# excamera/alfalfa

Hardware: NVIDIA H100
Metric: decode_throughput (higher is better)
Workload: dtype u8

## Files before the change

### alfalfa_b200/csrc/tokens.cu

```cuda
#include <cuda_runtime.h>
#include <stdint.h>
#include <stdlib.h>

#include "engine.h"
#include "tokens_core.cuh"

namespace vp8 {
namespace {

constexpr int kMaxCols = 1024;
template <int kTokWarps>
__global__ void __launch_bounds__(32 * kTokWarps) k_tokens(const uint8_t* ring, size_t stride, int first, int count,
                                                          int nslots, Geom g) {
  __shared__ __align__(16) uint8_t probs_all[kTokWarps][tok::kProbBytes];
  __shared__ uint16_t above_all[kTokWarps][kMaxCols];
  const int warp = threadIdx.x >> 5, lane = threadIdx.x & 31;
  const int job = blockIdx.x * kTokWarps + warp;
  if (job >= count) return;
  uint8_t* probs = probs_all[warp];
  uint16_t* above_nz = above_all[warp];
  const TokJob& J = *reinterpret_cast<const TokJob*>(ring + static_cast<size_t>((first + job) % nslots) * stride);
  for (int e = lane; e < tok::kProbEntries; e += 32) tok::expand_prob_entry(J.coef_probs, probs, e);
  for (int i = lane; i < g.mb_cols; i += 32) above_nz[i] = 0;
  __syncwarp();
  if (lane != 0) return;
  tok::decode_frame_tokens(J, g, probs, above_nz);
}

__global__ void __launch_bounds__(32) k_tokens_lockstep(const uint8_t* ring, size_t stride, int first, int count,
                                                         int nslots, Geom g) {
#ifdef VP8GPU_SIMT_EMUL
  uint8_t* const dyn = simt::dyn_smem();
#else
  extern __shared__ __align__(16) uint8_t dyn[];
#endif
  __shared__ tok::LockstepTables T;
  uint8_t* const P = dyn;
  uint16_t* const above = reinterpret_cast<uint16_t*>(dyn + 1056 * 32);
  const int lane = threadIdx.x;
  tok::fill_lockstep_tables(T, lane, 32);
  const int job = blockIdx.x * 32 + lane;
  const TokJob* J = job < count ? reinterpret_cast<const TokJob*>(ring + static_cast<size_t>((first + job) % nslots) * stride) : nullptr;
  if (J) {
    const uint32_t* src = reinterpret_cast<const uint32_t*>(J->coef_probs);
    for (int w = 0; w < 264; w++) {
      const uint32_t v = __ldg(src + w);
      P[(4 * w + 0) * 32 + lane] = v & 0xFF;
      P[(4 * w + 1) * 32 + lane] = (v >> 8) & 0xFF;
      P[(4 * w + 2) * 32 + lane] = (v >> 16) & 0xFF;
      P[(4 * w + 3) * 32 + lane] = v >> 24;
    }
  }
  __syncwarp();
  if (!J) return;
  tok::decode_frame_tokens_lockstep<32>(*J, g, T, P + lane, above + lane);
}

}

int launch_tokens(const uint8_t* ring, size_t stride, int first, int count, int nslots, const Geom& g, void* stream) {
  if (g.mb_cols > kMaxCols) return (int)cudaErrorInvalidValue;
  static const int warps = [] {
    const char* v = getenv("VP8GPU_TOK_WARPS");
    return v && atoi(v) == 8 ? 8 : (v && atoi(v) == 32 ? 32 : 1);
  }();
  cudaStream_t s = static_cast<cudaStream_t>(stream);
  if (warps == 32) {
    const size_t smem = 1056 * 32 + (size_t)g.mb_cols * 32 * sizeof(uint16_t);
    static const cudaError_t attr = cudaFuncSetAttribute(k_tokens_lockstep, cudaFuncAttributeMaxDynamicSharedMemorySize, 1056 * 32 + kMaxCols * 64);
    if (attr != cudaSuccess) return (int)attr;
    VP8_LAUNCH(k_tokens_lockstep, (count + 31) / 32, 32, smem, s)(ring, stride, first, count, nslots, g);
  }
  else if (warps == 8) VP8_LAUNCH(k_tokens<8>, (count + 7) / 8, 256, 0, s)(ring, stride, first, count, nslots, g);
  else VP8_LAUNCH(k_tokens<1>, count, 32, 0, s)(ring, stride, first, count, nslots, g);
  return (int)cudaGetLastError();
}

}
```

### alfalfa_b200/csrc/tokens_core.cuh

```cuda
#pragma once
#include <stdint.h>

#include "engine.h"

#ifdef __CUDACC__
#define TK_DEV __device__ __forceinline__
#define TK_CONST __constant__
#define TK_LDG(p) __ldg(p)
#define TK_LDCG(p) __ldcg(p)
#define TK_CLZ(x) __clz(x)
#else
#define TK_DEV inline __attribute__((always_inline))
#define TK_CONST static const
#define TK_LDG(p) (*(p))
#define TK_LDCG(p) (*(p))
#define TK_CLZ(x) __builtin_clz(x)
#endif

namespace vp8 {
namespace tok {

TK_CONST uint8_t c_band[16] = {0, 1, 2, 3, 6, 4, 5, 6, 6, 6, 6, 6, 6, 6, 6, 7};
TK_CONST uint8_t c_zigzag[16] = {0, 1, 4, 8, 5, 2, 3, 6, 9, 12, 13, 10, 7, 11, 14, 15};
TK_CONST uint8_t c_cat[5][11] = {{165, 145},
                                 {173, 148, 140},
                                 {176, 155, 140, 135},
                                 {180, 157, 141, 134, 130},
                                 {254, 254, 243, 230, 196, 177, 153, 140, 133, 130, 129}};

constexpr int kProbEntries = 4 * 8 * 3;
constexpr int kProbBytes = kProbEntries * 16;
struct alignas(16) Probs16 {
  uint32_t w[4];
  TK_DEV uint32_t at(int k) const { return (w[k >> 2] >> ((k & 3) * 8)) & 0xFF; }
};
TK_DEV void expand_prob_entry(const uint8_t* src, uint8_t* dst, int e) {
  for (int k = 0; k < 11; k++) dst[e * 16 + k] = src[e * 11 + k];
  for (int k = 11; k < 16; k++) dst[e * 16 + k] = 0;
}

#ifdef __CUDACC__
#define TK_BSWAP(x) __byte_perm((x), 0, 0x0123)
#else
#define TK_BSWAP(x) __builtin_bswap32(x)
#endif
struct LaneReader {
  const uint8_t* p;
  const uint8_t* end;
  uint64_t value;
  int nbits;
  uint32_t nxt;
  uint32_t range;
};
TK_DEV uint32_t lr_fetch(LaneReader& b) {
  uint32_t w = 0;
  if (b.p + 4 <= b.end) {
    w = TK_BSWAP(TK_LDG(reinterpret_cast<const uint32_t*>(b.p)));
  } else {
    for (int k = 0; k < 4; k++)
      if (b.p + k < b.end) w |= static_cast<uint32_t>(TK_LDG(b.p + k)) << (24 - 8 * k);
  }
  b.p += 4;
  return w;
}
TK_DEV void lr_refill(LaneReader& b) {
  b.value |= static_cast<uint64_t>(b.nxt) << (32 - b.nbits);
  b.nbits += 32;
  b.nxt = lr_fetch(b);
}
TK_DEV void lr_init(LaneReader& b, const uint8_t* data, uint32_t n) {
  b.p = data;
  b.end = data + n;
  b.value = 0;
  b.nbits = 0;
  b.range = 255;
  while ((reinterpret_cast<uintptr_t>(b.p) & 3) && b.p < b.end) {
    b.value |= static_cast<uint64_t>(TK_LDG(b.p++)) << (56 - b.nbits);
    b.nbits += 8;
  }
  if (b.p >= b.end) b.p = reinterpret_cast<const uint8_t*>((reinterpret_cast<uintptr_t>(b.p) + 3) & ~static_cast<uintptr_t>(3));
  b.nxt = lr_fetch(b);
  lr_refill(b);
  if (b.nbits <= 32) lr_refill(b);
}
TK_DEV int lr_decide(LaneReader& b, uint32_t prob) {
  const uint32_t split = 1 + (((b.range - 1) * prob) >> 8);
  uint32_t hi = static_cast<uint32_t>(b.value >> 32);
  const uint32_t big = split << 24;
  const int bit = hi >= big;
  const uint32_t r = bit ? b.range - split : split;
  hi -= bit ? big : 0u;
  const int shift = TK_CLZ(r) - 24;
  b.range = r << shift;
  b.value = ((static_cast<uint64_t>(hi) << 32) | static_cast<uint32_t>(b.value)) << shift;
  b.nbits -= shift;
  return bit;
}
TK_DEV void lr_ensure(LaneReader& b) {
  if (b.nbits <= 32) lr_refill(b);
}
TK_DEV int lr_get(LaneReader& b, uint32_t prob) {
  const int bit = lr_decide(b, prob);
  lr_ensure(b);
  return bit;
}

constexpr uint64_t kBandNibbles = 0x7666666665463210ull;
TK_DEV uint32_t band_off(int i) {
  return static_cast<uint32_t>((kBandNibbles >> (4 * (i & 15))) & 15) * 48;
}
TK_DEV Probs16 ld_probs(const uint8_t* p) { return *reinterpret_cast<const Probs16*>(p); }

TK_DEV int parse_block(LaneReader& br, const uint8_t* tp, int ctx, int i, uint32_t tag, vp8gpu_token*& out) {
  lr_ensure(br);
  Probs16 P = ld_probs(tp + band_off(i) + ctx * 16);
  if (!lr_decide(br, P.at(0))) return 0;
  int nz = 0;
  for (;;) {
    lr_ensure(br);
    const uint32_t next = band_off(i + 1);
    const Probs16 Pz = ld_probs(tp + next);
    if (!lr_decide(br, P.at(1))) {
      if (++i == 16) return nz;
      P = Pz;
      continue;
    }
    int v;
    Probs16 Pn;
    if (!lr_decide(br, P.at(2))) {
      Pn = ld_probs(tp + next + 16);
      v = 1;
    } else {
      Pn = ld_probs(tp + next + 32);
      lr_ensure(br);
      if (!lr_decide(br, P.at(3))) {
        if (!lr_decide(br, P.at(4))) v = 2;
        else v = 3 + lr_decide(br, P.at(5));
      } else {
        int cat, n, base;
        if (!lr_decide(br, P.at(6))) {
          if (!lr_decide(br, P.at(7))) {
            cat = 0, n = 0, base = 5 + lr_decide(br, 159);
          } else {
            cat = 0, n = 2, base = 7;
          }
        } else if (!lr_decide(br, P.at(8))) {
          if (!lr_decide(br, P.at(9))) cat = 1, n = 3, base = 11;
          else cat = 2, n = 4, base = 19;
        } else {
          if (!lr_decide(br, P.at(10))) cat = 3, n = 5, base = 35;
          else cat = 4, n = 11, base = 67;
        }
        int inc = 0;
        for (int k = 0; k < n; k++) {
          lr_ensure(br);
          inc = (inc << 1) + lr_decide(br, c_cat[cat][k]);
        }
        v = base + inc;
      }
      lr_ensure(br);
    }
    if (lr_decide(br, 128)) v = -v;
    *out++ = tag | (static_cast<uint32_t>(c_zigzag[i]) << 16) | static_cast<uint16_t>(v);
    nz = 1;
    if (++i == 16) return 1;
    P = Pn;
    if (!lr_decide(br, P.at(0))) return 1;
  }
}

TK_DEV void decode_frame_tokens(const TokJob& J, const Geom& g, const uint8_t* probs, uint16_t* above_nz) {
  LaneReader parts[8];
  const int nparts = static_cast<int>(J.nparts);
  for (int i = 0; i < nparts; i++) lr_init(parts[i], J.bits + J.part_off[i], J.part_len[i]);

  vp8gpu_mb* const mbs = J.mbs;
  vp8gpu_token* const t_begin = J.tokens;
  vp8gpu_token* t = t_begin;
  const vp8gpu_token* const t_limit = t_begin + J.tok_cap;
  uint32_t overflow = 0;
  const uint8_t* const coef_y_after_y2 = probs + 0 * 384;
  const uint8_t* const coef_y2 = probs + 1 * 384;
  const uint8_t* const coef_uv = probs + 2 * 384;
  const uint8_t* const coef_y_full = probs + 3 * 384;

  const uint32_t* rec = reinterpret_cast<const uint32_t*>(mbs);
  uint32_t w1 = TK_LDCG(rec + 1), w2 = TK_LDCG(rec + 2);
  const int n_mbs = g.mb_cols * g.mb_rows;
  int idx = 0;
  for (int row = 0; row < g.mb_rows; row++) {
    unsigned left_nz = 0;
    LaneReader tr = parts[row & (nparts - 1)];
    for (int col = 0; col < g.mb_cols; col++, idx++) {
      const uint32_t cur1 = w1, cur2 = w2;
      if (idx + 1 < n_mbs) {
        w1 = TK_LDCG(rec + 8 * (idx + 1) + 1);
        w2 = TK_LDCG(rec + 8 * (idx + 1) + 2);
      }
      const int y_mode = (cur1 >> 16) & 0xFF;
      const bool skip = (cur2 >> 24) & VP8GPU_MB_SKIP;
      const bool has_y2 = y_mode != VP8GPU_B_PRED && y_mode != VP8GPU_SPLITMV;
      unsigned a_nz = above_nz[col];
      vp8gpu_token* const t0 = t;
      if (skip) {
        const unsigned keep = has_y2 ? 0u : 0x100u;
        a_nz &= keep;
        left_nz &= keep;
      } else if (t + 400 > t_limit) {
        overflow = 1;
        a_nz = 0;
        left_nz = 0;
      } else {
        const uint8_t* y_probs = coef_y_full;
        int first = 0;
        if (has_y2) {
          const int ctx = ((a_nz >> 8) & 1) + ((left_nz >> 8) & 1);
          const unsigned nz = parse_block(tr, coef_y2, ctx, 0, VP8GPU_BLK_Y2 << 20, t);
          a_nz = (a_nz & ~0x100u) | (nz << 8);
          left_nz = (left_nz & ~0x100u) | (nz << 8);
          y_probs = coef_y_after_y2;
          first = 1;
        }
#pragma unroll 1
        for (int b = 0; b < 24; b++) {
          int bx, by;
          const uint8_t* tp;
          int f;
          if (b < 16) {
            bx = b & 3, by = b >> 2, tp = y_probs, f = first;
          } else {
            const int sh = 4 + 2 * ((b - 16) >> 2);
            bx = sh + (b & 1), by = sh + ((b >> 1) & 1), tp = coef_uv, f = 0;
          }
          const int ctx = ((a_nz >> bx) & 1) + ((left_nz >> by) & 1);
          const unsigned nz = parse_block(tr, tp, ctx, f, static_cast<uint32_t>(b) << 20, t);
          a_nz = (a_nz & ~(1u << bx)) | (nz << bx);
          left_nz = (left_nz & ~(1u << by)) | (nz << by);
        }
      }
      above_nz[col] = static_cast<uint16_t>(a_nz);
      uint32_t* wr = reinterpret_cast<uint32_t*>(mbs) + 8 * idx;
      wr[0] = static_cast<uint32_t>(t0 - t_begin);
      wr[1] = (cur1 & 0xFFFF0000u) | static_cast<uint32_t>(t - t0);
      wr[2] = cur2 & ~(static_cast<uint32_t>(VP8GPU_MB_SKIP) << 24);
    }
    parts[row & (nparts - 1)] = tr;
  }
  J.result[0] = static_cast<uint32_t>(t - t_begin);
  if (overflow) J.result[1] = 1;
}


constexpr int kNodeExtra = 11, kNodeSign = 12, kNodeEnd = 13;
#define TK_T(next, setv, zero, cat) static_cast<uint16_t>((next) | ((setv) << 4) | ((zero) << 8) | ((cat) << 9))
TK_CONST uint16_t c_trans[22] = {
    TK_T(kNodeEnd, 0, 0, 0),  TK_T(1, 0, 0, 0),
    TK_T(1, 0, 1, 0),         TK_T(2, 0, 0, 0),
    TK_T(kNodeSign, 1, 0, 0), TK_T(3, 0, 0, 0),
    TK_T(4, 0, 0, 0),         TK_T(6, 0, 0, 0),
    TK_T(kNodeSign, 2, 0, 0), TK_T(5, 0, 0, 0),
    TK_T(kNodeSign, 3, 0, 0), TK_T(kNodeSign, 4, 0, 0),
    TK_T(7, 0, 0, 0),         TK_T(8, 0, 0, 0),
    TK_T(kNodeExtra, 0, 0, 1), TK_T(kNodeExtra, 0, 0, 2),
    TK_T(9, 0, 0, 0),         TK_T(10, 0, 0, 0),
    TK_T(kNodeExtra, 0, 0, 3), TK_T(kNodeExtra, 0, 0, 4),
    TK_T(kNodeExtra, 0, 0, 5), TK_T(kNodeExtra, 0, 0, 6),
};
#undef TK_T
TK_CONST uint8_t c_cat_base[7] = {0, 5, 7, 11, 19, 35, 67};
TK_CONST uint8_t c_cat_bits[7] = {0, 1, 2, 3, 4, 5, 11};
TK_CONST uint8_t c_cat_prob[7][11] = {{0},
                                      {159},
                                      {165, 145},
                                      {173, 148, 140},
                                      {176, 155, 140, 135},
                                      {180, 157, 141, 134, 130},
                                      {254, 254, 243, 230, 196, 177, 153, 140, 133, 130, 129}};

struct LockstepTables {
  uint16_t trans[22];
  uint8_t band[16], zigzag[16], cat_base[8], cat_bits[8], cat_prob[7][11];
};
TK_DEV void fill_lockstep_tables(LockstepTables& T, int lane, int nlanes) {
  for (int k = lane; k < 22; k += nlanes) T.trans[k] = c_trans[k];
  for (int k = lane; k < 16; k += nlanes) {
    T.band[k] = c_band[k];
    T.zigzag[k] = c_zigzag[k];
  }
  for (int k = lane; k < 7; k += nlanes) {
    T.cat_base[k] = c_cat_base[k];
    T.cat_bits[k] = c_cat_bits[k];
    for (int j = 0; j < 11; j++) T.cat_prob[k][j] = c_cat_prob[k][j];
  }
}


template <int LS>
TK_DEV void decode_frame_tokens_lockstep(const TokJob& J, const Geom& g, const LockstepTables& T, const uint8_t* P,
                                         uint16_t* above) {
  for (int c = 0; c < g.mb_cols; c++) above[c * LS] = 0;
  LaneReader parts[8];
  const int nparts = static_cast<int>(J.nparts);
  for (int k = 0; k < nparts; k++) lr_init(parts[k], J.bits + J.part_off[k], J.part_len[k]);
  uint8_t* const mbs = reinterpret_cast<uint8_t*>(J.mbs);
  vp8gpu_token* const t_begin = J.tokens;
  vp8gpu_token* t = t_begin;
  vp8gpu_token* t0 = t_begin;
  const vp8gpu_token* const t_limit = t_begin + J.tok_cap;
  uint32_t overflow = 0;
  const int n_mbs = g.mb_cols * g.mb_rows;
  const int n_words = (n_mbs + 15) >> 4;
  uint32_t info = n_words > 0 ? TK_LDG(J.mbinfo) : 0u, info_next = n_words > 1 ? TK_LDG(J.mbinfo + 1) : 0u;

  LaneReader tr = parts[0];
  int idx = 0, col = 0, row = 0;
  unsigned a_nz = 0, left_nz = 0;
  int bq = 0, last_y_type = 0, first_y = 0;
  int has_y2_cur = 0;
  int type_off = 0, bx = 0, by = 0;
  int i = 0, ctx = 0, node = kNodeEnd, nz = 0;
  int v = 0, acc = 0, cat = 0, nrem = 0, extra_k = 0;
  bool need_mb = true;
  bool done = n_mbs == 0;

  while (!done) {
    if (node == kNodeEnd) {
      if (!need_mb) {
        a_nz = (a_nz & ~(1u << bx)) | (static_cast<unsigned>(nz) << bx);
        left_nz = (left_nz & ~(1u << by)) | (static_cast<unsigned>(nz) << by);
        bq++;
        if (bq == 24) {
          above[col * LS] = static_cast<uint16_t>(a_nz);
          uint8_t* rec = mbs + 32 * static_cast<size_t>(idx);
          *reinterpret_cast<uint32_t*>(rec) = static_cast<uint32_t>(t0 - t_begin);
          *reinterpret_cast<uint16_t*>(rec + 4) = static_cast<uint16_t>(t - t0);
          rec[11] = static_cast<uint8_t>(has_y2_cur ? VP8GPU_MB_HAS_Y2 : 0);
          idx++;
          col++;
          need_mb = true;
        }
      }
      while (need_mb && !done) {
        if (idx == n_mbs) {
          done = true;
          break;
        }
        if (col == g.mb_cols) {
          parts[row & (nparts - 1)] = tr;
          row++;
          col = 0;
          left_nz = 0;
          tr = parts[row & (nparts - 1)];
        }
        const unsigned bits2 = (info >> (2 * (idx & 15))) & 3u;
        if ((idx & 15) == 15) {
          info = info_next;
          const int nw = (idx >> 4) + 2;
          info_next = nw < n_words ? TK_LDG(J.mbinfo + nw) : 0u;
        }
        const bool skip = (bits2 & VP8GPU_MB_SKIP) != 0;
        const bool has_y2 = (bits2 & VP8GPU_MB_HAS_Y2) != 0;
        has_y2_cur = has_y2;
        a_nz = above[col * LS];
        t0 = t;
        bool settled = false;
        if (skip) {
          const unsigned keep = has_y2 ? 0u : 0x100u;
          a_nz &= keep;
          left_nz &= keep;
          settled = true;
        } else if (t + 400 > t_limit) {
          overflow = 1;
          a_nz = 0;
          left_nz = 0;
          settled = true;
        }
        if (settled) {
          above[col * LS] = static_cast<uint16_t>(a_nz);
          uint8_t* rec = mbs + 32 * static_cast<size_t>(idx);
          *reinterpret_cast<uint32_t*>(rec) = static_cast<uint32_t>(t0 - t_begin);
          *reinterpret_cast<uint16_t*>(rec + 4) = 0;
          rec[11] = static_cast<uint8_t>(has_y2 ? VP8GPU_MB_HAS_Y2 : 0);
          idx++;
          col++;
          continue;
        }
        need_mb = false;
        bq = has_y2 ? -1 : 0;
        last_y_type = has_y2 ? 0 : 3;
        first_y = has_y2 ? 1 : 0;
      }
      if (done) break;
      if (bq < 0) {
        type_off = 1 * 264, bx = 8, by = 8, i = 0;
      } else if (bq < 16) {
        type_off = last_y_type * 264, bx = bq & 3, by = bq >> 2, i = first_y;
      } else {
        const int sh = 4 + 2 * ((bq - 16) >> 2);
        type_off = 2 * 264, bx = sh + (bq & 1), by = sh + ((bq >> 1) & 1), i = 0;
      }
      ctx = ((a_nz >> bx) & 1) + ((left_nz >> by) & 1);
      node = 0;
      nz = 0;
    }

    const int tree_node = node <= 10 ? node : 0;
    const uint32_t p_tree = P[(type_off + T.band[i & 15] * 33 + ctx * 11 + tree_node) * LS];
    const uint32_t p_extra = T.cat_prob[cat][extra_k];
    const uint32_t prob = node <= 10 ? p_tree : (node == kNodeExtra ? p_extra : 128u);
    const int bit = lr_get(tr, prob);

    if (node <= 10) {
      const uint32_t e = T.trans[node * 2 + bit];
      node = e & 15;
      const int setv = (e >> 4) & 15;
      v = setv ? setv : v;
      if ((e >> 8) & 1) {
        i++;
        ctx = 0;
        if (i == 16) node = kNodeEnd;
      }
      const int c = (e >> 9) & 7;
      if (c) {
        cat = c;
        nrem = T.cat_bits[c];
        acc = 0;
        extra_k = 0;
      }
    } else if (node == kNodeExtra) {
      acc = (acc << 1) + bit;
      extra_k++;
      if (--nrem == 0) {
        v = T.cat_base[cat] + acc;
        extra_k = 0;
        node = kNodeSign;
      }
    } else {
      const int sv = bit ? -v : v;
      const int blk = bq < 0 ? VP8GPU_BLK_Y2 : bq;
      *t++ = (static_cast<uint32_t>(blk) << 20) | (static_cast<uint32_t>(T.zigzag[i]) << 16) | static_cast<uint16_t>(sv);
      nz = 1;
      ctx = v == 1 ? 1 : 2;
      i++;
      node = i == 16 ? kNodeEnd : 0;
    }
  }
  J.result[0] = static_cast<uint32_t>(t - t_begin);
  if (overflow) J.result[1] = 1;
}

}
}
```

Measured before the change: 10770.

## Rework boolean decoder arithmetic with split 32-bit state and shared-memory prob loads

Rewrites the bool-decoder state from a 64-bit value plus 8-bit range into two 32-bit halves and a range pre-shifted by 16 bits. The split threshold is now computed in a single multiply-add, normalisation uses bfind and a funnel shift, and the 64-bit shifts on the serial decode path are dropped. Probability tables are addressed through 32-bit shared-memory addresses with explicit ld.shared.v4 loads instead of generic pointers, and the refill check is moved after the prefetch load. The aim is a shorter dependency chain per decoded bit in this latency-bound serial token parser, at the cost of inline PTX and tricky arithmetic equivalence.

```diff
diff --git a/alfalfa_b200/csrc/tokens.cu b/alfalfa_b200/csrc/tokens.cu
--- a/alfalfa_b200/csrc/tokens.cu
+++ b/alfalfa_b200/csrc/tokens.cu
@@ -14,7 +14,7 @@
                                                           int nslots, Geom g) {
   __shared__ __align__(16) uint8_t probs_all[kTokWarps][tok::kProbBytes];
   __shared__ uint16_t above_all[kTokWarps][kMaxCols];
-  const int warp = threadIdx.x >> 5, lane = threadIdx.x & 31;
+  const int warp = kTokWarps == 1 ? 0 : threadIdx.x >> 5, lane = threadIdx.x & 31;
   const int job = blockIdx.x * kTokWarps + warp;
   if (job >= count) return;
   uint8_t* probs = probs_all[warp];
diff --git a/alfalfa_b200/csrc/tokens_core.cuh b/alfalfa_b200/csrc/tokens_core.cuh
--- a/alfalfa_b200/csrc/tokens_core.cuh
+++ b/alfalfa_b200/csrc/tokens_core.cuh
@@ -41,16 +41,18 @@
 
 #ifdef __CUDACC__
 #define TK_BSWAP(x) __byte_perm((x), 0, 0x0123)
+#define TK_FUNNEL_L(lo, hi, s) __funnelshift_l((lo), (hi), (s))
 #else
 #define TK_BSWAP(x) __builtin_bswap32(x)
+#define TK_FUNNEL_L(lo, hi, s) static_cast<uint32_t>(((static_cast<uint64_t>(hi) << 32) | (lo)) << (s) >> 32)
 #endif
 struct LaneReader {
   const uint8_t* p;
   const uint8_t* end;
-  uint64_t value;
+  uint32_t hi, lo;
   int nbits;
   uint32_t nxt;
-  uint32_t range;
+  uint32_t rng16;
 };
 TK_DEV uint32_t lr_fetch(LaneReader& b) {
   uint32_t w = 0;
@@ -64,35 +66,50 @@
   return w;
 }
 TK_DEV void lr_refill(LaneReader& b) {
-  b.value |= static_cast<uint64_t>(b.nxt) << (32 - b.nbits);
+  const uint64_t v = (static_cast<uint64_t>(b.nxt) << 32) >> b.nbits;
+  b.hi |= static_cast<uint32_t>(v >> 32);
+  b.lo = static_cast<uint32_t>(v);
   b.nbits += 32;
   b.nxt = lr_fetch(b);
 }
 TK_DEV void lr_init(LaneReader& b, const uint8_t* data, uint32_t n) {
   b.p = data;
   b.end = data + n;
-  b.value = 0;
+  uint64_t value = 0;
   b.nbits = 0;
-  b.range = 255;
+  b.rng16 = 255u << 16;
   while ((reinterpret_cast<uintptr_t>(b.p) & 3) && b.p < b.end) {
-    b.value |= static_cast<uint64_t>(TK_LDG(b.p++)) << (56 - b.nbits);
+    value |= static_cast<uint64_t>(TK_LDG(b.p++)) << (56 - b.nbits);
     b.nbits += 8;
   }
+  b.hi = static_cast<uint32_t>(value >> 32);
+  b.lo = static_cast<uint32_t>(value);
   if (b.p >= b.end) b.p = reinterpret_cast<const uint8_t*>((reinterpret_cast<uintptr_t>(b.p) + 3) & ~static_cast<uintptr_t>(3));
   b.nxt = lr_fetch(b);
   lr_refill(b);
   if (b.nbits <= 32) lr_refill(b);
 }
+#ifndef TK_ON_DECISION
+#define TK_ON_DECISION()
+#endif
 TK_DEV int lr_decide(LaneReader& b, uint32_t prob) {
-  const uint32_t split = 1 + (((b.range - 1) * prob) >> 8);
-  uint32_t hi = static_cast<uint32_t>(b.value >> 32);
-  const uint32_t big = split << 24;
-  const int bit = hi >= big;
-  const uint32_t r = bit ? b.range - split : split;
-  hi -= bit ? big : 0u;
-  const int shift = TK_CLZ(r) - 24;
-  b.range = r << shift;
-  b.value = ((static_cast<uint64_t>(hi) << 32) | static_cast<uint32_t>(b.value)) << shift;
+  TK_ON_DECISION();
+  const uint32_t M = 0xFFFFFFu;
+  const uint32_t t = b.rng16 * prob + ((256u - prob) << 16);
+  const int bit = (b.hi | M) >= t;
+  const uint32_t r = bit ? ((b.rng16 << 8) | M) - t : t;
+  const uint32_t h = bit ? b.hi - (t & ~M) : b.hi;
+#ifdef __CUDACC__
+  int shift;
+  asm("bfind.shiftamt.u32 %0, %1;" : "=r"(shift) : "r"(r));
+  const uint32_t r16 = __byte_perm(r, 0, 0x4344);
+#else
+  const int shift = TK_CLZ(r);
+  const uint32_t r16 = (r >> 24) << 16;
+#endif
+  b.rng16 = r16 << shift;
+  b.hi = TK_FUNNEL_L(b.lo, h, shift);
+  b.lo <<= shift;
   b.nbits -= shift;
   return bit;
 }
@@ -109,17 +126,34 @@
 TK_DEV uint32_t band_off(int i) {
   return static_cast<uint32_t>((kBandNibbles >> (4 * (i & 15))) & 15) * 48;
 }
-TK_DEV Probs16 ld_probs(const uint8_t* p) { return *reinterpret_cast<const Probs16*>(p); }
-
-TK_DEV int parse_block(LaneReader& br, const uint8_t* tp, int ctx, int i, uint32_t tag, vp8gpu_token*& out) {
+#ifdef __CUDACC__
+typedef uint32_t ProbAddr;
+TK_DEV ProbAddr prob_addr(const uint8_t* p) {
+  uint32_t a;
+  asm volatile("mov.u32 %0, %1;" : "=r"(a) : "r"(static_cast<uint32_t>(__cvta_generic_to_shared(p))));
+  return a;
+}
+TK_DEV Probs16 ld_probs(ProbAddr a) {
+  Probs16 P;
+  asm volatile("ld.shared.v4.u32 {%0, %1, %2, %3}, [%4];"
+               : "=r"(P.w[0]), "=r"(P.w[1]), "=r"(P.w[2]), "=r"(P.w[3]) : "r"(a));
+  return P;
+}
+#else
+typedef const uint8_t* ProbAddr;
+TK_DEV ProbAddr prob_addr(const uint8_t* p) { return p; }
+TK_DEV Probs16 ld_probs(ProbAddr p) { return *reinterpret_cast<const Probs16*>(p); }
+#endif
+
+TK_DEV int parse_block(LaneReader& br, ProbAddr tp, int ctx, int i, uint32_t tag, vp8gpu_token*& out) {
   lr_ensure(br);
   Probs16 P = ld_probs(tp + band_off(i) + ctx * 16);
   if (!lr_decide(br, P.at(0))) return 0;
   int nz = 0;
   for (;;) {
-    lr_ensure(br);
     const uint32_t next = band_off(i + 1);
     const Probs16 Pz = ld_probs(tp + next);
+    lr_ensure(br);
     if (!lr_decide(br, P.at(1))) {
       if (++i == 16) return nz;
       P = Pz;
@@ -179,10 +213,10 @@
   vp8gpu_token* t = t_begin;
   const vp8gpu_token* const t_limit = t_begin + J.tok_cap;
   uint32_t overflow = 0;
-  const uint8_t* const coef_y_after_y2 = probs + 0 * 384;
-  const uint8_t* const coef_y2 = probs + 1 * 384;
-  const uint8_t* const coef_uv = probs + 2 * 384;
-  const uint8_t* const coef_y_full = probs + 3 * 384;
+  const ProbAddr coef_y_after_y2 = prob_addr(probs);
+  const ProbAddr coef_y2 = coef_y_after_y2 + 1 * 384;
+  const ProbAddr coef_uv = coef_y_after_y2 + 2 * 384;
+  const ProbAddr coef_y_full = coef_y_after_y2 + 3 * 384;
 
   const uint32_t* rec = reinterpret_cast<const uint32_t*>(mbs);
   uint32_t w1 = TK_LDCG(rec + 1), w2 = TK_LDCG(rec + 2);
@@ -211,7 +245,7 @@
         a_nz = 0;
         left_nz = 0;
       } else {
-        const uint8_t* y_probs = coef_y_full;
+        ProbAddr y_probs = coef_y_full;
         int first = 0;
         if (has_y2) {
           const int ctx = ((a_nz >> 8) & 1) + ((left_nz >> 8) & 1);
@@ -224,7 +258,7 @@
 #pragma unroll 1
         for (int b = 0; b < 24; b++) {
           int bx, by;
-          const uint8_t* tp;
+          ProbAddr tp;
           int f;
           if (b < 16) {
             bx = b & 3, by = b >> 2, tp = y_probs, f = first;
```

Result: faster. 11570, median of 6 (+7.5%).
